# semchan/DCT_Pruning

Measured on NVIDIA B200. Metric: dct_importance_score_images_per_s, higher is better.
Workload: dtype bf16 hi/lo split of fp32 on tcgen05 (fp32 accumulate), fp64 cross-image sums

## Files before the change

### dct_pruning_b200/csrc/dctp.cu

```cuda
#include <cmath>
#include <cstdarg>
#include <cstdio>
#include <cstdlib>
#include <cstring>
#include <map>
#include <mutex>
#include <utility>
#include <vector>

#include "../../include/dctp.h"
#include "score_simt.cuh"
#include "score_large.cuh"
#include "score_tmem.cuh"
#include "score_stack.cuh"
#include "score_kron.cuh"
#include "score_umma.cuh"
#include "topk.cuh"
#include "gather.cuh"
#include "score_alt.cuh"

namespace {

using namespace dctp;

// ... 101 lines not shown
    auto key = std::make_pair(N, KP);
    auto it = g.umma.find(key);
    if (it != g.umma.end()) { out = it->second; return DCTP_OK; }
    const int Ms = (N + 7) / 8 * 8, J = KP / Ms;
    std::vector<uint16_t> hi(static_cast<size_t>(KP) * KP, 0), lo(hi.size(), 0);
    for (int j = 0; j < J; ++j)
        for (int v = 0; v < N; ++v)
            for (int w = 0; w < N; ++w)
                split_bf16(dct_coef(v, w, N), hi[(size_t)(j * Ms + v) * KP + j * Ms + w], lo[(size_t)(j * Ms + v) * KP + j * Ms + w]);
    UmmaBasis b;
    CUDA_TRY(cudaMalloc(&b.hi, hi.size() * 2));
    CUDA_TRY(cudaMalloc(&b.lo, lo.size() * 2));
    CUDA_TRY(cudaMemcpy(b.hi, hi.data(), hi.size() * 2, cudaMemcpyHostToDevice));
    CUDA_TRY(cudaMemcpy(b.lo, lo.data(), lo.size() * 2, cudaMemcpyHostToDevice));
    const int G = 128 / Ms, MT = G * J, NN = N * N;
    if ((MT * NN) % 4 == 0) {
        b.vpe = (N % 4 == 0) ? 1 : (N % 2 == 0) ? 2 : 4;
        b.tile_vec = MT * NN / 4;
        const int step = 4 / b.vpe;
        std::vector<uint16_t> tab(static_cast<size_t>(b.tile_vec) * b.vpe + 8, 0);
        for (int v = 0; v < b.tile_vec; ++v)
            for (int s = 0; s < b.vpe; ++s) {
                const int e = 4 * v + s * step, t = e / NN, r = e % NN;
                tab[(size_t)v * b.vpe + s] =
                    static_cast<uint16_t>(detail::kmajor_off((t / J) * Ms + r / N, (t % J) * Ms + r % N, 128));
            }
        CUDA_TRY(cudaMalloc(&b.scatter, tab.size() * 2));
        CUDA_TRY(cudaMemcpy(b.scatter, tab.data(), tab.size() * 2, cudaMemcpyHostToDevice));
    }
    g.umma[key] = b;
    out = b;
    return DCTP_OK;
}

inline int t_n1max(int N) { return N <= 32 ? 32 : 64; }
inline int t_groups(int N) { return N <= 8 ? 4 : N <= 16 ? 2 : 1; }

int get_t_basis(int N, TBasis& out) {
    auto it = g.tmem.find(N);
    if (it != g.tmem.end()) { out = it->second; return DCTP_OK; }
    const int Ms = (N + 7) / 8 * 8, G = 128 / Ms, NN = N * N, rows = t_n1max(N), J = t_groups(N);
    std::vector<uint32_t> ahi(128 * 64, 0), alo(128 * 64, 0);
    std::vector<uint16_t> chi(64 * 64, 0), clo(64 * 64, 0);
    for (int gI = 0; gI < G; ++gI)
        for (int v = 0; v < N; ++v)
            for (int w = 0; w < N; ++w) {
                uint16_t h, l;
                split_bf16(dct_coef(v, w, N), h, l);
                const int row = gI * Ms + v, k = gI * N + w;
                ahi[row * 64 + k / 2] |= static_cast<uint32_t>(h) << (16 * (k & 1));
                alo[row * 64 + k / 2] |= static_cast<uint32_t>(l) << (16 * (k & 1));
            }
    for (int rep = 0; rep < (Ms == 8 ? 2 : 1); ++rep)
        for (int u = 0; u < N; ++u)
            for (int h = 0; h < N; ++h) split_bf16(dct_coef(u, h, N), chi[(rep * 8 + u) * 64 + rep * 8 + h], clo[(rep * 8 + u) * 64 + rep * 8 + h]);
    TBasis b;
    b.vpe = (N % 4 == 0) ? 1 : (N % 2 == 0) ? 2 : 4;
    b.tile_vec = G * J * NN / 4;
    const int step = 4 / b.vpe;
    std::vector<uint16_t> tab(static_cast<size_t>(b.tile_vec) * b.vpe + 8, 0);
    for (int v = 0; v < b.tile_vec; ++v)
        for (int sI = 0; sI < b.vpe; ++sI) {
            const int e = 4 * v + sI * step, t = e / NN, r = e % NN, gI = t / J, j = t % J;
            tab[(size_t)v * b.vpe + sI] = static_cast<uint16_t>(detail::kmajor_off(j * Ms + r / N, gI * N + r % N, rows));
        }
    CUDA_TRY(cudaMalloc(&b.a_hi, ahi.size() * 4));
    CUDA_TRY(cudaMalloc(&b.a_lo, alo.size() * 4));
    CUDA_TRY(cudaMalloc(&b.c_hi, chi.size() * 2));
    CUDA_TRY(cudaMalloc(&b.c_lo, clo.size() * 2));
    CUDA_TRY(cudaMalloc(&b.scatter, tab.size() * 2));
    CUDA_TRY(cudaMemcpy(b.a_hi, ahi.data(), ahi.size() * 4, cudaMemcpyHostToDevice));
    CUDA_TRY(cudaMemcpy(b.a_lo, alo.data(), alo.size() * 4, cudaMemcpyHostToDevice));
    CUDA_TRY(cudaMemcpy(b.c_hi, chi.data(), chi.size() * 2, cudaMemcpyHostToDevice));
    CUDA_TRY(cudaMemcpy(b.c_lo, clo.data(), clo.size() * 2, cudaMemcpyHostToDevice));
    CUDA_TRY(cudaMemcpy(b.scatter, tab.data(), tab.size() * 2, cudaMemcpyHostToDevice));
    g.tmem[N] = b;
    out = b;
    return DCTP_OK;
}

inline int stack_kp(int N) { return (N + 15) / 16 * 16; }
inline int stack_sets(int kp) { return kp <= 32 ? 64 / kp : 1; }
inline int stack_g(int kp) { return kp == 16 ? 8 : kp == 32 ? 4 : 2; }
bool stack_shape_supported(int N) { return N >= 10 && N <= 64 && (N % 2) == 0 && (N <= 32 || (N % 4) == 0); }

int get_stack_basis(int N, StackBasis& out) {
    auto it = g.stack.find(N);
    if (it != g.stack.end()) { out = it->second; return DCTP_OK; }
    using S = StackSmem;
    const int KP = stack_kp(N), J = stack_sets(KP), G = stack_g(KP), NN = N * N, Np = (N + 7) / 8 * 8, MT = G * J;
    std::vector<uint32_t> img(128 * 32, 0);
    for (int lane = 0; lane < 128; ++lane) {
        const int q = lane >> 5, part = (lane >> 4) & 1, r = lane & 15;
        const int set = J == 4 ? q : J == 2 ? q >> 1 : 0;
        const int v = J == 4 ? r : J == 2 ? 16 * (q & 1) + r : 16 * q + r;
        if (v >= N) continue;
        for (int w = 0; w < N; ++w) {
            uint16_t h, l;
            split_bf16(dct_coef(v, w, N), h, l);
            const int k = set * KP + w;
            img[lane * 32 + k / 2] |= static_cast<uint32_t>(part ? l : h) << (16 * (k & 1));
        }
    }
    std::vector<uint8_t> chi(S::C2_HALF, 0), clo(S::C2_HALF, 0);
    for (int u = 0; u < N; ++u)
        for (int h = 0; h < N; ++h) {
            uint16_t hh, ll;
            split_bf16(dct_coef(u, h, N), hh, ll);
            const size_t off = static_cast<size_t>(h / 8) * S::LBO2 + u * 16 + (h % 8) * 2;
            std::memcpy(&chi[off], &hh, 2);
            std::memcpy(&clo[off], &ll, 2);
        }
    StackBasis b;
    b.kp = KP;
    b.vec = (N % 4) == 0 ? 4 : 2;
    b.tile_vec = MT * NN / 4;
    const int pieces = b.vec == 4 ? 1 : 2;
    std::vector<uint16_t> tab(static_cast<size_t>(b.tile_vec) * pieces + 8, 0);
    auto fill = [&](uint32_t lbo) {
        for (int f = 0; f < b.tile_vec; ++f)
            for (int pc = 0; pc < pieces; ++pc) {
                const int e = 4 * f + 2 * pc, m = e / NN, rem = e % NN, h = rem / N, w = rem % N, gI = m / J, set = m % J;
                const int n = gI * Np + h, k = set * KP + w;
                tab[static_cast<size_t>(f) * pieces + pc] = static_cast<uint16_t>((k / 8) * lbo + n * 16 + (k % 8) * 2);
            }
    };
    auto store_wavefronts = [&]() {
        long long total = 0;
        const int width = b.vec == 4 ? 2 : 1, lanes = b.vec == 4 ? 16 : 32;
        for (int f0 = 0; f0 < b.tile_vec; f0 += lanes)
            for (int pc = 0; pc < pieces; ++pc) {
                int cnt[32] = {0}, worst = 0;
                for (int t = 0; t < lanes && f0 + t < b.tile_vec; ++t)
                    for (int w = 0; w < width; ++w) {
                        const int bank = (tab[static_cast<size_t>(f0 + t) * pieces + pc] / 4 + w) % 32;
                        if (++cnt[bank] > worst) worst = cnt[bank];
                    }
                total += worst;
            }
        return total;
    };
    long long best = -1;
    for (uint32_t u = 0; u < 8; ++u) {
        fill(2048u + 16u * u);
        const long long wf = store_wavefronts();
        if (best < 0 || wf < best) { best = wf; b.lbo1 = 2048u + 16u * u; }
    }
    fill(b.lbo1);
    b.table_bytes = static_cast<uint32_t>((static_cast<size_t>(b.tile_vec) * pieces * 2 + 15) / 16 * 16);
    if (b.table_bytes > S::TABLE_MAX) return fail(DCTP_E_UNSUPPORTED, "stacked-basis kernel: offset table of side %d does not fit", N);
    CUDA_TRY(cudaMalloc(&b.a_img, img.size() * 4));
    CUDA_TRY(cudaMalloc(&b.c2_hi, chi.size()));
    CUDA_TRY(cudaMalloc(&b.c2_lo, clo.size()));
    CUDA_TRY(cudaMalloc(&b.table, tab.size() * 2));
    CUDA_TRY(cudaMemcpy(b.a_img, img.data(), img.size() * 4, cudaMemcpyHostToDevice));
    CUDA_TRY(cudaMemcpy(b.c2_hi, chi.data(), chi.size(), cudaMemcpyHostToDevice));
    CUDA_TRY(cudaMemcpy(b.c2_lo, clo.data(), clo.size(), cudaMemcpyHostToDevice));
    CUDA_TRY(cudaMemcpy(b.table, tab.data(), tab.size() * 2, cudaMemcpyHostToDevice));
    g.stack[N] = b;
    out = b;
    return DCTP_OK;
}

constexpr int STACK_CFGS = 8, STACK_VARIANTS = 10;
typedef void (*StackKernel)(const ScoreTensorMaps, const StackArgs);
template <bool TRACE, int NCONV, int NE1G = 1, int NE2G = 2>
StackKernel stack_kernel_of(int v) {
    switch (v) {
        case 0: return score_stack_kernel<16, 4, NCONV, NE1G, 2, NE2G, 2, TRACE>;
        case 1: return score_stack_kernel<16, 2, NCONV, NE1G, 2, NE2G, 2, TRACE>;
        case 2: return score_stack_kernel<32, 4, NCONV, NE1G, 2, NE2G, 3, TRACE>;
        case 3: return score_stack_kernel<32, 4, NCONV, NE1G, 2, NE2G, 4, TRACE>;
        case 4: return score_stack_kernel<32, 2, NCONV, NE1G, 2, NE2G, 3, TRACE>;
        case 5: return score_stack_kernel<32, 2, NCONV, NE1G, 2, NE2G, 4, TRACE>;
        case 6: return score_stack_kernel<48, 4, NCONV, NE1G, 2, NE2G, 5, TRACE>;
        case 7: return score_stack_kernel<48, 4, NCONV, NE1G, 2, NE2G, 6, TRACE>;
        case 8: return score_stack_kernel<64, 4, NCONV, NE1G, 2, NE2G, 7, TRACE>;
        default: return score_stack_kernel<64, 4, NCONV, NE1G, 2, NE2G, 8, TRACE>;
    }
}
bool stack_cfg_valid(int cfg) { return cfg == 4 || cfg == 6 || cfg == 7; }
StackKernel stack_kernel_fn(int cfg, int v) {
    switch (cfg) {
        case 6: return stack_kernel_of<true, 8>(v);
        case 7: return stack_kernel_of<false, 12>(v);
        default: return stack_kernel_of<false, 8>(v);
    }
}
const void* stack_kernel_ptr(int cfg, int v) { return reinterpret_cast<const void*>(stack_kernel_fn(cfg, v)); }
int stack_threads(int cfg) { return (cfg == 7 ? 31 : 27) * 32; }
int stack_variant(int KP, int vec, int np8) {
    if (KP == 16) return vec == 4 ? 0 : 1;
    if (KP == 32) return (vec == 4 ? 2 : 4) + (np8 == 4 ? 1 : 0);
    if (KP == 48) return np8 == 6 ? 7 : 6;
    return np8 == 8 ? 9 : 8;
}

typedef CUresult (*EncodeTiledFn)(CUtensorMap*, CUtensorMapDataType, cuuint32_t, void*, const cuuint64_t*, const cuuint64_t*, const cuuint32_t*,
                                  const cuuint32_t*, CUtensorMapInterleave, CUtensorMapSwizzle, CUtensorMapL2promotion, CUtensorMapFloatOOBfill);

template <typename Args>
cudaError_t launch_score_tma(void (*kern)(const ScoreTensorMaps, const Args), int grid, int block, size_t smem, cudaStream_t stream,
                             const ScoreTensorMaps& maps, const Args& args);

struct SiteDesc { const float* first; int B; int c_count; double* accum; };

int encode_flat_map(CUtensorMap& map, const float* first, long long total_elems, int box_rows) {
    std::memset(&map, 0, sizeof map);
    const long long rows = total_elems / 32;
    if (rows <= 0) return DCTP_OK;
    cuuint64_t gdim[2] = {32, static_cast<cuuint64_t>(rows)};
    cuuint64_t gstr[1] = {128};
    cuuint32_t box[2] = {32, static_cast<cuuint32_t>(box_rows)}, estr[2] = {1, 1};
    const CUresult r = reinterpret_cast<EncodeTiledFn>(g.encode_tiled)(
        &map, CU_TENSOR_MAP_DATA_TYPE_FLOAT32, 2, const_cast<float*>(first), gdim, gstr, box, estr, CU_TENSOR_MAP_INTERLEAVE_NONE,
        CU_TENSOR_MAP_SWIZZLE_NONE, CU_TENSOR_MAP_L2_PROMOTION_L2_128B, CU_TENSOR_MAP_FLOAT_OOB_FILL_NONE);
    if (r != CUDA_SUCCESS) return fail(DCTP_E_CUDA, "cuTensorMapEncodeTiled failed (%d) for %lld rows, box %d", (int)r, rows, box_rows);
    return DCTP_OK;
}

int fill_segments(ScoreSegments& seg, const SiteDesc* sites, int n, int NN, int maps_per_tile) {
    seg.n_seg = n;
    int tiles = 0;
    for (int i = 0; i < n; ++i) {
        seg.tile0[i] = tiles;
        seg.n_maps[i] = sites[i].B * sites[i].c_count;
        seg.c_count[i] = sites[i].c_count;
        seg.total_elems[i] = static_cast<long long>(seg.n_maps[i]) * NN;
        seg.x[i] = sites[i].first;
        seg.accum[i] = sites[i].accum;
        tiles += (seg.n_maps[i] + maps_per_tile - 1) / maps_per_tile;
    }
    for (int i = n; i <= SCORE_MAX_SEG; ++i) seg.tile0[i] = tiles;
    return tiles;
}

int launch_stack(const SiteDesc* sites, int n, int N, float* energy_out, float* coeff_out, cudaStream_t stream) {
    StackBasis basis;
    int rc = get_stack_basis(N, basis);
    if (rc) return rc;
    StackArgs a;
    std::memset(&a, 0, sizeof a);
    const int KP = basis.kp, J = stack_sets(KP);
    a.N = N; a.NN = N * N; a.Np = (N + 7) / 8 * 8; a.G = stack_g(KP); a.MT = a.G * J;
    a.ncols = a.G * a.Np;
    a.tile_elems = a.MT * a.NN; a.tile_rows = a.tile_elems / 32; a.tile_vec = basis.tile_vec;
    a.num_tiles = fill_segments(a.seg, sites, n, a.NN, a.MT);
    a.idesc1 = umma::make_idesc_bf16(128, a.ncols, false, false);
    a.idesc2 = umma::make_idesc_bf16(128, KP, false, false);
    a.lbo1 = basis.lbo1;
    a.a_img = basis.a_img; a.c2_hi = basis.c2_hi; a.c2_lo = basis.c2_lo; a.table = basis.table; a.table_bytes = basis.table_bytes;
    a.energy_out = n == 1 ? energy_out : nullptr; a.dump = n == 1 ? coeff_out : nullptr; a.status = g.status;
    ScoreTensorMaps maps;
    for (int i = 0; i < n; ++i)
        if ((rc = encode_flat_map(maps.m[i], sites[i].first, a.seg.total_elems[i], a.tile_rows))) return rc;
    for (int i = n; i < SCORE_MAX_SEG; ++i) maps.m[i] = maps.m[0];
    int grid = g.sm_count < a.num_tiles ? g.sm_count : a.num_tiles;
    const size_t smem = StackSmem::TOTAL;
    const bool v4 = basis.vec == 4;
    static long long* trace_buf = nullptr;
    const bool tracing = std::getenv("DCTP_S_TRACE") != nullptr;
    if (tracing) {
        if (!trace_buf) CUDA_TRY(cudaMalloc(&trace_buf, 64 * sizeof(long long)));
        CUDA_TRY(cudaMemset(trace_buf, 0, 64 * sizeof(long long)));
        a.trace = trace_buf;
    }
    const int variant = stack_variant(KP, v4 ? 4 : 2, a.Np / 8);
    const int cfg = (a.energy_out || a.dump || tracing) ? 6 : g.stack_cfg ? g.stack_cfg : 7;
    CUDA_TRY(launch_score_tma(stack_kernel_fn(cfg, variant), grid, stack_threads(cfg), smem, stream, maps, a));
    note_kernel("score_stack_kernel<KP=%d,VEC=%d,cfg%d> (tcgen05, stacked hi/lo basis in TMEM, TMA tile ring, warp specialised)", KP, basis.vec, cfg);
    if (tracing) {
        long long h[64];
        CUDA_TRY(cudaMemcpy(h, trace_buf, sizeof h, cudaMemcpyDeviceToHost));
        const double nt = h[14] > 0 ? double(h[14]) : 1.0;
        fprintf(stderr, "[dctp trace] stack N=%d cfg %d, CTA 0, %lld tiles, cycles per tile | producer: wait slot %.0f | converter: wait Bx free %.0f, "
                        "wait TMA %.0f, convert %.0f, fence+arrive %.0f | issuer 1: wait Bx %.0f, wait D1 free %.0f, issue %.0f | issuer 2: wait A2 %.0f, "
                        "wait D2 free %.0f, issue %.0f | epi1 (first group, per tile of the CTA): wait D1 %.0f, wait A2 free %.0f, work %.0f | "
                        "epi2: wait D2 %.0f, TMEM loads %.0f, sums+shuffles %.0f, atomics %.0f\n",
                N, cfg, h[14], h[0] / nt, h[16] / nt, h[17] / nt, h[18] / nt, h[19] / nt, h[8] / nt, h[9] / nt, h[10] / nt, h[40] / nt,
                h[41] / nt, h[42] / nt, h[24] / nt, h[25] / nt, h[26] / nt, h[32] / nt, h[34] / nt, h[35] / nt, h[33] / nt);
        fprintf(stderr, "[dctp trace] CTA 0, ns since kernel entry: TMEM + barriers ready %lld, bases staged and dependency wait over %lld, tile loop %lld\n", h[52], h[53], h[51]);
        fprintf(stderr, "[dctp trace] tile loop of CTA 0: %lld SM cycles in %lld ns = %.0f MHz, %.0f cycles per tile\n", h[50], h[51],
                h[51] > 0 ? 1e3 * double(h[50]) / double(h[51]) : 0.0, double(h[50]) / nt);
    }
    g.launches += 1;
    CUDA_TRY(cudaGetLastError());
    return DCTP_OK;
}

int get_kron_basis(int N, KronBasis& out) {
    auto it = g.kron.find(N);
    if (it != g.kron.end()) { out = it->second; return DCTP_OK; }
    using S = StackSmem;
    std::vector<uint8_t> hi(S::C2_HALF, 0), lo(S::C2_HALF, 0);
    for (int u = 0; u < N; ++u)
        for (int v = 0; v < N; ++v)
            for (int h = 0; h < N; ++h)
                for (int w = 0; w < N; ++w) {
                    uint16_t hh, ll;
                    split_bf16(dct_coef(u, h, N) * dct_coef(v, w, N), hh, ll);
                    const int n = u * N + v, k = h * N + w;
                    const size_t off = static_cast<size_t>(k / 8) * S::LBO2 + n * 16 + (k % 8) * 2;
                    std::memcpy(&hi[off], &hh, 2);
                    std::memcpy(&lo[off], &ll, 2);
                }
    KronBasis b;
    CUDA_TRY(cudaMalloc(&b.hi, hi.size()));
    CUDA_TRY(cudaMalloc(&b.lo, lo.size()));
    CUDA_TRY(cudaMemcpy(b.hi, hi.data(), hi.size(), cudaMemcpyHostToDevice));
    CUDA_TRY(cudaMemcpy(b.lo, lo.data(), lo.size(), cudaMemcpyHostToDevice));
    g.kron[N] = b;
    out = b;
    return DCTP_OK;
}

int launch_kron(const SiteDesc* sites, int n, int N, float* energy_out, float* coeff_out, cudaStream_t stream) {
    KronBasis basis;
    int rc = get_kron_basis(N, basis);
    if (rc) return rc;
    KronArgs a;
    std::memset(&a, 0, sizeof a);
    const int NN = N * N, K2 = (NN + 15) / 16 * 16;
    const bool even = (N % 2) == 0;
    a.N = N; a.NN = NN;
    a.idesc = umma::make_idesc_bf16(128, K2, false, false);
    a.k_hi = basis.hi; a.k_lo = basis.lo;
    a.energy_out = n == 1 ? energy_out : nullptr; a.dump = n == 1 ? coeff_out : nullptr; a.status = g.status;
    if (even) {
        a.sub_tiles = N == 8 ? 1 : 2;
        a.row_floats = NN + (((NN / 4) % 2) == 0 ? 4 : 0);
        a.tile_maps = 128 * a.sub_tiles;
        a.box_rows = a.tile_maps;
        a.tile_bytes = static_cast<uint32_t>(a.tile_maps) * a.row_floats * 4u;
    } else {
        a.sub_tiles = N == 7 ? 1 : N == 5 ? 2 : 4;
        a.row_floats = NN;
        a.tile_maps = 128 * a.sub_tiles;
        a.box_rows = a.tile_maps * NN / 32;
        a.tile_bytes = static_cast<uint32_t>(a.box_rows) * 128u;
    }
    a.num_tiles = fill_segments(a.seg, sites, n, NN, a.tile_maps);
    ScoreTensorMaps maps;
    for (int i = 0; i < n; ++i) {
        if (even) {
            std::memset(&maps.m[i], 0, sizeof(CUtensorMap));
            cuuint64_t gdim[2] = {static_cast<cuuint64_t>(NN), static_cast<cuuint64_t>(a.seg.n_maps[i])};
            cuuint64_t gstr[1] = {static_cast<cuuint64_t>(NN) * 4};
            cuuint32_t box[2] = {static_cast<cuuint32_t>(a.row_floats), static_cast<cuuint32_t>(a.tile_maps)}, estr[2] = {1, 1};
            const CUresult r = reinterpret_cast<EncodeTiledFn>(g.encode_tiled)(
                &maps.m[i], CU_TENSOR_MAP_DATA_TYPE_FLOAT32, 2, const_cast<float*>(sites[i].first), gdim, gstr, box, estr,
// ... 889 lines not shown
```

### dct_pruning_b200/csrc/score_stack.cuh

```cuda
#pragma once
#include <cuda.h>
#include "score_umma.cuh"

namespace dctp {

constexpr int SCORE_MAX_SEG = 16;

struct ScoreSegments {
    int n_seg;
    int tile0[SCORE_MAX_SEG + 1];
    int n_maps[SCORE_MAX_SEG], c_count[SCORE_MAX_SEG];
    long long total_elems[SCORE_MAX_SEG];
    const float* x[SCORE_MAX_SEG];
    double* accum[SCORE_MAX_SEG];
};
struct ScoreTensorMaps { CUtensorMap m[SCORE_MAX_SEG]; };

struct StackArgs {
    ScoreSegments seg;
    int N, NN, Np;
    int G, MT;
    int ncols;
    int tile_elems, tile_rows, tile_vec, num_tiles;
    uint32_t idesc1, idesc2;
    uint32_t lbo1;
    const uint32_t* a_img;
    const uint8_t* c2_hi;
    const uint8_t* c2_lo;
    const uint16_t* table;
    uint32_t table_bytes;
    float* energy_out;
    float* dump;
    int* status;
    long long* trace;
};

struct StackSmem {
    static constexpr uint32_t NSTG = 3, STG_STRIDE = 32768;
    static constexpr uint32_t LBO1_MAX = 128 * 16 + 16 * 7;
    static constexpr uint32_t BX_HALF = 8 * LBO1_MAX;
    static constexpr uint32_t LBO2 = 64 * 16 + 16;
    static constexpr uint32_t C2_HALF = 8 * LBO2;
    static constexpr uint32_t OFF_BX = NSTG * STG_STRIDE;
    static constexpr uint32_t NBX = 3;
    static constexpr uint32_t OFF_C2 = OFF_BX + 2 * NBX * BX_HALF;
    static constexpr uint32_t OFF_TABLE = OFF_C2 + 2 * C2_HALF;
    static constexpr uint32_t TABLE_MAX = 8192;
    static constexpr uint32_t OFF_RED = OFF_TABLE + TABLE_MAX;
    static constexpr uint32_t OFF_BARS = OFF_RED + 256;
    static constexpr uint32_t OFF_SLOT = OFF_BARS + 256;
    static constexpr uint32_t TOTAL = OFF_SLOT + 128;
};


template <int KP, int VEC, int NCONV, int NE1G, int NCG, int NE2G = 1, int NP8 = 0, bool TRACE = false>
__global__ void __launch_bounds__((NCONV + 8 * NE1G + 4 * NE2G + 3) * 32, 1) score_stack_kernel(const __grid_constant__ ScoreTensorMaps tmaps, const __grid_constant__ StackArgs a) {
    using S = StackSmem;
    using namespace umma;
    constexpr int J = KP <= 32 ? 64 / KP : 1;
    constexpr int K1S = J * KP / 16, K2S = KP / 16;
    constexpr int G = KP == 16 ? 8 : KP == 32 ? 4 : 2, T2 = G / 2;
    constexpr uint32_t W_E1 = NCONV, W_E2 = NCONV + 8 * NE1G, W_PROD = W_E2 + 4 * NE2G, W_MMA = W_PROD + 1, W_MMA2 = W_PROD + 2, NT = (W_MMA2 + 1) * 32;
    constexpr uint32_t NCT = NCONV * 32 / NCG;
    constexpr uint32_t NBXK = KP == 32 ? 2u : 3u;
    constexpr uint32_t TM_A = 0, TM_D1 = 32;
    const uint32_t d1_stride = a.ncols <= 112 ? 112u : 128u;
    const uint32_t TM_A2 = TM_D1 + 2 * d1_stride, TM_D2 = TM_A2 + 128;
    const uint32_t nb2 = TM_D2 + 128 <= 512 ? 2u : 1u;
    const uint32_t STEP1 = (2 * a.lbo1) >> 4;
    constexpr uint32_t STEP2 = (2 * S::LBO2) >> 4;

    extern __shared__ __align__(1024) uint8_t smem[];
    const uint32_t tid = threadIdx.x, warp = __shfl_sync(0xffffffffu, tid >> 5, 0), lane = tid & 31;
    uint8_t* stg = smem;
    uint8_t* bx = smem + S::OFF_BX;
    uint8_t* c2 = smem + S::OFF_C2;
    const uint8_t* tab = smem + S::OFF_TABLE;
    float* red = reinterpret_cast<float*>(smem + S::OFF_RED);
    uint64_t* bars = reinterpret_cast<uint64_t*>(smem + S::OFF_BARS);
    uint64_t* stg_full = bars;
    uint64_t* stg_free = bars + 3;
    uint64_t* bx_full = bars + 6;
    uint64_t* bx_free = bars + 9;
    uint64_t* d1_full = bars + 12;
    uint64_t* d1_free = bars + 14;
    uint64_t* a2_full = bars + 16;
    uint64_t* a2_free = bars + 18;
    uint64_t* d2_full = bars + 20;
    uint64_t* d2_free = bars + 22;
    uint32_t* tmem_slot = reinterpret_cast<uint32_t*>(smem + S::OFF_SLOT);

    long long tr_entry = 0;
    if (TRACE && a.trace != nullptr && blockIdx.x == 0 && threadIdx.x == 0) asm volatile("mov.u64 %0, %%globaltimer;" : "=l"(tr_entry));
    if (warp == W_MMA) tmem_alloc<512>(tmem_slot);
    if (tid == 0) {
        for (int s = 0; s < 3; ++s) { mbar_init(stg_full + s, 1); mbar_init(stg_free + s, NCONV / NCG); }
        for (int b = 0; b < (int)S::NBX; ++b) { mbar_init(bx_full + b, NCONV / NCG); mbar_init(bx_free + b, 1); }
        for (int b = 0; b < 2; ++b) {
            mbar_init(d1_full + b, 1); mbar_init(d1_free + b, 8);
            mbar_init(a2_full + b, 8); mbar_init(a2_free + b, 1);
            mbar_init(d2_full + b, 1); mbar_init(d2_free + b, 4);
        }
        mbar_init_fence();
    }
    if (warp == W_PROD && lane == 0) tma_prefetch_desc(&tmaps.m[0]);
    tc_fence_before_sync();
    __syncthreads();
    tc_fence_after_sync();
    const uint32_t tmem = *tmem_slot;
    launch_dependents();
    if (TRACE && a.trace != nullptr && blockIdx.x == 0 && tid == 0) { long long t_; asm volatile("mov.u64 %0, %%globaltimer;" : "=l"(t_)); a.trace[52] = t_ - tr_entry; }
    if (warp != W_PROD) {
        const uint32_t ptid = tid < W_PROD * 32 ? tid : tid - 32;
        constexpr uint32_t PNT = NT - 32;
        static_assert(2 * PNT * 16 >= S::C2_HALF && PNT * 16 >= S::TABLE_MAX, "prologue loads are unrolled for these sizes");
        uint4 c2h[2], c2l[2], tb = make_uint4(0, 0, 0, 0), ai[8];
#pragma unroll
        for (int i = 0; i < 2; ++i) {
            const uint32_t off = (ptid + i * PNT) * 16;
            if (off < S::C2_HALF) {
                c2h[i] = *reinterpret_cast<const uint4*>(a.c2_hi + off);
                c2l[i] = *reinterpret_cast<const uint4*>(a.c2_lo + off);
            }
        }
        if (ptid * 16 < a.table_bytes) tb = *reinterpret_cast<const uint4*>(reinterpret_cast<const uint8_t*>(a.table) + ptid * 16);
        if (warp < 4) {
#pragma unroll
            for (int i = 0; i < 8; ++i) ai[i] = reinterpret_cast<const uint4*>(a.a_img + tid * 32)[i];
        }
        for (uint32_t off = ptid * 16; off < 2 * S::NBX * S::BX_HALF; off += PNT * 16) *reinterpret_cast<uint4*>(bx + off) = make_uint4(0, 0, 0, 0);
#pragma unroll
        for (int i = 0; i < 2; ++i) {
            const uint32_t off = (ptid + i * PNT) * 16;
            if (off < S::C2_HALF) {
                *reinterpret_cast<uint4*>(c2 + off) = c2h[i];
                *reinterpret_cast<uint4*>(c2 + S::C2_HALF + off) = c2l[i];
            }
        }
        if (ptid * 16 < a.table_bytes) *reinterpret_cast<uint4*>(smem + S::OFF_TABLE + ptid * 16) = tb;
        if (warp < 4) {
#pragma unroll
            for (int part = 0; part < 2; ++part) {
                uint32_t v[16];
#pragma unroll
                for (int i = 0; i < 4; ++i) {
                    const uint4 q4 = ai[4 * part + i];
                    v[4 * i] = q4.x; v[4 * i + 1] = q4.y; v[4 * i + 2] = q4.z; v[4 * i + 3] = q4.w;
                }
                tmem_st16(tmem + ((warp * 32u) << 16) + TM_A + part * 16, v);
            }
            tmem_st_wait();
// ... 130 lines not shown
                if (!tail) ++it;
                continue;
            }
            const uint32_t b = n % NBXK, s = it % S::NSTG;
            TR_START();
            {
                bool ok = true;
                if (n >= NBXK) ok = mbar_wait(bx_free + b, ((n / NBXK) - 1u) & 1u);
                TR_ADD(tr0);
                if (ok && !tail) ok = mbar_wait(stg_full + s, (it / S::NSTG) & 1u);
                TR_ADD(tr1);
                if (!ok) { dead = true; break; }
            }
            uint8_t* hi = bx + b * 2 * S::BX_HALF;
            uint8_t* lo = hi + S::BX_HALF;
            auto emit = [&](uint32_t o, const float4 v) {
                uint32_t h0, l0, h1, l1;
                split2_packed(pack2(__float_as_uint(v.x), __float_as_uint(v.y)), h0, l0);
                split2_packed(pack2(__float_as_uint(v.z), __float_as_uint(v.w)), h1, l1);
                if constexpr (VEC == 4) {
                    *reinterpret_cast<uint2*>(hi + o) = make_uint2(h0, h1);
                    *reinterpret_cast<uint2*>(lo + o) = make_uint2(l0, l1);
                } else {
                    const uint32_t o0 = o & 0xFFFFu, o1 = o >> 16;
                    *reinterpret_cast<uint32_t*>(hi + o0) = h0;
                    *reinterpret_cast<uint32_t*>(lo + o0) = l0;
                    *reinterpret_cast<uint32_t*>(hi + o1) = h1;
                    *reinterpret_cast<uint32_t*>(lo + o1) = l1;
                }
            };
            auto entry = [&](int f) {
                return VEC == 4 ? static_cast<uint32_t>(reinterpret_cast<const uint16_t*>(tab)[f]) : reinterpret_cast<const uint32_t*>(tab)[f];
            };
            if (!tail) {
                const float4* src = reinterpret_cast<const float4*>(stg + s * S::STG_STRIDE);
                constexpr int CB = 3;
                int f0 = ctid;
                for (; f0 + (int)NCT * (CB - 1) < a.tile_vec - (a.tile_vec % (int)NCT) ; f0 += NCT * CB) {
                    float4 v[CB];
                    uint32_t o[CB];
#pragma unroll
                    for (int i = 0; i < CB; ++i) { v[i] = src[f0 + (int)NCT * i]; o[i] = entry(f0 + (int)NCT * i); }
#pragma unroll
                    for (int i = 0; i < CB; ++i) emit(o[i], v[i]);
                }
                {
                    float4 v[CB];
                    uint32_t o[CB];
#pragma unroll
                    for (int i = 0; i < CB; ++i) {
                        const int f = f0 + (int)NCT * i;
                        if (f < a.tile_vec) { v[i] = src[f]; o[i] = entry(f); }
                    }
#pragma unroll
                    for (int i = 0; i < CB; ++i)
                        if (f0 + (int)NCT * i < a.tile_vec) emit(o[i], v[i]);
                }
                TR_ADD(tr2);
                __syncwarp();
                if (lane == 0) mbar_arrive(stg_free + s);
                ++it;
            } else {
                const long long e0 = static_cast<long long>(tile - a.seg.tile0[sg]) * a.tile_elems, total = a.seg.total_elems[sg];
                const float* xs = a.seg.x[sg];
                for (int f = ctid; f < a.tile_vec; f += NCT) {
                    const long long e = e0 + 4ll * f;
                    float4 v;
                    v.x = e + 0 < total ? xs[e + 0] : 0.f;
                    v.y = e + 1 < total ? xs[e + 1] : 0.f;
                    v.z = e + 2 < total ? xs[e + 2] : 0.f;
                    v.w = e + 3 < total ? xs[e + 3] : 0.f;
                    emit(entry(f), v);
                }
            }
            fence_async_smem();
            __syncwarp();
            if (lane == 0) mbar_arrive(bx_full + b);
            TR_ADD(tr3);
        }
        TR_FLUSH(16);
    } else if (warp < W_E2) {
        const uint32_t q = warp & 3u, s = ((warp - W_E1) >> 2) & 1u, eg = (warp - W_E1) >> 3;
        const uint32_t lane_q = (q * 32u) << 16, lane_s = (q * 32u + s * 16u) << 16;
        const int np8 = NP8 ? NP8 : (a.Np >> 3);
        tr_me = tr_on && warp == W_E1 && lane == 0;
        auto convert16 = [&](const uint32_t (&za)[8], const uint32_t (&zb)[8], uint32_t dst_hi, uint32_t dst_lo) {
            uint32_t h[4], l[4];
#pragma unroll
            for (int i = 0; i < 4; ++i)
                split2_packed(add2_packed(pack2(za[2 * i], za[2 * i + 1]), pack2(zb[2 * i], zb[2 * i + 1])), h[i], l[i]);
            tmem_st_frag8(dst_hi, h);
            tmem_st_frag8(dst_lo, l);
        };
        uint32_t n = eg;
        for (int tile = first + (int)eg * stride; tile < a.num_tiles; tile += NE1G * stride, n += NE1G) {
            const uint32_t b = n & 1u;
            const uint32_t d1 = tmem + TM_D1 + b * d1_stride;
            TR_START();
            {
                bool ok = true;
                ok = mbar_wait(d1_full + b, (n >> 1) & 1u);
                TR_ADD(tr0);
                if (ok && n >= 2) ok = mbar_wait(a2_free + b, ((n >> 1) - 1u) & 1u);
                TR_ADD(tr1);
                if (!ok) { dead = true; break; }
            }
            tc_fence_after_sync();
            constexpr int CPT = KP / 16, NCH = T2 * CPT;
#pragma unroll
            for (int ch0 = 0; ch0 < NCH; ch0 += 2) {
                uint32_t za[16], zb[16];
#pragma unroll
                for (int k = 0; k < 2; ++k) {
                    const int ch = ch0 + k;
                    if (ch < NCH) {
                        const int t = ch / CPT, c8 = 2 * (ch % CPT);
                        const uint32_t src_a = d1 + lane_q + (2 * t + s) * a.Np + c8 * 8, src_b = src_a + (16u << 16);
                        if (c8 + 2 <= np8) {
                            tmem_ld_frag16(src_a, reinterpret_cast<uint32_t (&)[8]>(za[8 * k]));
                            tmem_ld_frag16(src_b, reinterpret_cast<uint32_t (&)[8]>(zb[8 * k]));
                        } else if (c8 < np8) {
                            tmem_ld_frag8(src_a, reinterpret_cast<uint32_t (&)[4]>(za[8 * k]));
                            tmem_ld_frag8(src_b, reinterpret_cast<uint32_t (&)[4]>(zb[8 * k]));
                        }
                    }
                }
                tmem_ld_wait();
                if (ch0 + 2 >= NCH) {
                    tc_fence_before_sync();
                    __syncwarp();
                    if (lane == 0) mbar_arrive(d1_free + b);
                }
#pragma unroll
                for (int k = 0; k < 2; ++k) {
                    const int ch = ch0 + k;
                    if (ch < NCH) {
                        const int t = ch / CPT, c8 = 2 * (ch % CPT);
                        const uint32_t dst_hi = tmem + TM_A2 + b * 64 + t * KP + lane_s + c8 * 4, dst_lo = dst_hi + KP / 2;
                        if (c8 + 2 <= np8) {
                            convert16(reinterpret_cast<const uint32_t (&)[8]>(za[8 * k]), reinterpret_cast<const uint32_t (&)[8]>(zb[8 * k]), dst_hi, dst_lo);
                        } else if (c8 < np8) {
                            uint32_t h[2], l[2];
#pragma unroll
                            for (int i = 0; i < 2; ++i)
                                split2_packed(add2_packed(pack2(za[8 * k + 2 * i], za[8 * k + 2 * i + 1]), pack2(zb[8 * k + 2 * i], zb[8 * k + 2 * i + 1])),
                                              h[i], l[i]);
                            tmem_st_frag4(dst_hi, h[0], h[1]);
                            tmem_st_frag4(dst_lo, l[0], l[1]);
                        }
                    }
                }
            }
            tmem_st_wait();
            tc_fence_before_sync();
            __syncwarp();
            if (lane == 0) mbar_arrive(a2_full + b);
            TR_ADD(tr2);
        }
        TR_FLUSH(24);
    } else if (warp < W_PROD) {
        const uint32_t q = warp & 3u, eg2 = (warp - W_E2) >> 2, et = tid - (W_E2 + 4 * eg2) * 32;
        const uint32_t lane_q = (q * 32u) << 16;
        const uint32_t s = lane >> 4, r = lane & 15u;
        const uint32_t my_set = J == 4 ? q : J == 2 ? (q >> 1) : 0u;
        const uint32_t my_v = J == 4 ? r : J == 2 ? 16u * (q & 1u) + r : 16u * q + r;
        uint32_t n = eg2;
        int sg = 0, chan_sg = -1;
        uint32_t chan0 = 0, chan_step = 0;
        tr_me = tr_on && warp == W_E2 && lane == 0;
        for (int tile = first + (int)eg2 * stride; tile < a.num_tiles; tile += NE2G * stride, n += NE2G) {
            seg_of(tile, sg);
            const uint32_t C = static_cast<uint32_t>(a.seg.c_count[sg]), seg_maps = static_cast<uint32_t>(a.seg.n_maps[sg]);
            double* const accum = a.seg.accum[sg];
            const uint32_t pb = n & 1u, b2 = nb2 == 2 ? pb : 0u;
            TR_START();
            if (!mbar_wait(d2_full + pb, (n >> 1) & 1u)) { dead = true; break; }
            TR_ADD(tr0);
            tc_fence_after_sync();
            const uint32_t d2 = tmem + TM_D2 + b2 * 64 + lane_q;
            const uint32_t m0 = static_cast<uint32_t>(tile - a.seg.tile0[sg]) * a.MT;
            if (sg != chan_sg) {
                chan_sg = sg;
                chan0 = m0 % C;
                chan_step = (static_cast<uint32_t>(NE2G * stride) * static_cast<uint32_t>(a.MT)) % C;
            } else {
                chan0 += chan_step;
                if (chan0 >= C) chan0 -= C;
            }
            float e[T2];
            constexpr int TOT = T2 * KP, HALF = TOT >= 32 ? 32 : TOT;
            float part[4] = {0.f, 0.f, 0.f, 0.f};
#pragma unroll
            for (int c0 = 0; c0 < TOT; c0 += HALF) {
                uint32_t z[HALF];
#pragma unroll
                for (int c = 0; c < HALF; c += 16)
                    if (c0 + c < TOT) tmem_ld16(d2 + c0 + c, reinterpret_cast<uint32_t (&)[16]>(z[c]));
                tmem_ld_wait();
                if (c0 + HALF >= TOT) {
                    tc_fence_before_sync();
                    __syncwarp();
                    if (lane == 0) mbar_arrive(d2_free + pb);
                    TR_ADD(tr2);
                }
#pragma unroll
                for (int c = 0; c < HALF; c += 16) {
                    if (c0 + c < TOT) {
                        const int t = (c0 + c) / KP;
                        float p0 = 0.f, p1 = 0.f, p2 = 0.f, p3 = 0.f;
#pragma unroll
                        for (int i = 0; i < 4; ++i) {
                            p0 = fmaf(__uint_as_float(z[c + i]), __uint_as_float(z[c + i]), p0);
                            p1 = fmaf(__uint_as_float(z[c + 4 + i]), __uint_as_float(z[c + 4 + i]), p1);
                            p2 = fmaf(__uint_as_float(z[c + 8 + i]), __uint_as_float(z[c + 8 + i]), p2);
                            p3 = fmaf(__uint_as_float(z[c + 12 + i]), __uint_as_float(z[c + 12 + i]), p3);
                        }
                        const float p = (p0 + p1) + (p2 + p3);
                        if (T2 == 4) part[t] += p;
                        else if (T2 == 2) part[t] += p;
                        else part[0] += p;
                        if (TRACE && a.dump != nullptr) {
                            const uint32_t m = m0 + (2 * t + s) * J + my_set;
                            const int u0 = (c0 + c) - t * KP;
                            if (m < seg_maps && my_v < (uint32_t)a.N)
#pragma unroll
                                for (int i = 0; i < 16; ++i)
                                    if (u0 + i < a.N) a.dump[static_cast<long long>(m) * a.NN + (u0 + i) * a.N + my_v] = __uint_as_float(z[c + i]);
                        }
                    }
                }
            }
// ... 71 lines not shown
```

Baseline: 122,200.

## Tighten TMEM map pitch per side length and specialise stacked kernel per pitch

New measurement: 126,200 (median of 6 runs). 1.03x the previous value.

```diff
diff --git a/dct_pruning_b200/csrc/dctp.cu b/dct_pruning_b200/csrc/dctp.cu
--- a/dct_pruning_b200/csrc/dctp.cu
+++ b/dct_pruning_b200/csrc/dctp.cu
@@ -207,13 +207,14 @@
 inline int stack_kp(int N) { return (N + 15) / 16 * 16; }
 inline int stack_sets(int kp) { return kp <= 32 ? 64 / kp : 1; }
 inline int stack_g(int kp) { return kp == 16 ? 8 : kp == 32 ? 4 : 2; }
+inline int stack_pitch(int N) { const int r = stack_kp(N) == 16 ? 16 : 16 / stack_g(stack_kp(N)); return (N + r - 1) / r * r; }
 bool stack_shape_supported(int N) { return N >= 10 && N <= 64 && (N % 2) == 0 && (N <= 32 || (N % 4) == 0); }
 
 int get_stack_basis(int N, StackBasis& out) {
     auto it = g.stack.find(N);
     if (it != g.stack.end()) { out = it->second; return DCTP_OK; }
     using S = StackSmem;
-    const int KP = stack_kp(N), J = stack_sets(KP), G = stack_g(KP), NN = N * N, Np = (N + 7) / 8 * 8, MT = G * J;
+    const int KP = stack_kp(N), J = stack_sets(KP), G = stack_g(KP), NN = N * N, Np = stack_pitch(N), MT = G * J;
     std::vector<uint32_t> img(128 * 32, 0);
     for (int lane = 0; lane < 128; ++lane) {
         const int q = lane >> 5, part = (lane >> 4) & 1, r = lane & 15;
@@ -287,21 +288,25 @@
     return DCTP_OK;
 }
 
-constexpr int STACK_CFGS = 8, STACK_VARIANTS = 10;
+constexpr int STACK_CFGS = 8, STACK_VARIANTS = 14;
 typedef void (*StackKernel)(const ScoreTensorMaps, const StackArgs);
 template <bool TRACE, int NCONV, int NE1G = 1, int NE2G = 2>
 StackKernel stack_kernel_of(int v) {
     switch (v) {
-        case 0: return score_stack_kernel<16, 4, NCONV, NE1G, 2, NE2G, 2, TRACE>;
-        case 1: return score_stack_kernel<16, 2, NCONV, NE1G, 2, NE2G, 2, TRACE>;
-        case 2: return score_stack_kernel<32, 4, NCONV, NE1G, 2, NE2G, 3, TRACE>;
-        case 3: return score_stack_kernel<32, 4, NCONV, NE1G, 2, NE2G, 4, TRACE>;
-        case 4: return score_stack_kernel<32, 2, NCONV, NE1G, 2, NE2G, 3, TRACE>;
-        case 5: return score_stack_kernel<32, 2, NCONV, NE1G, 2, NE2G, 4, TRACE>;
-        case 6: return score_stack_kernel<48, 4, NCONV, NE1G, 2, NE2G, 5, TRACE>;
-        case 7: return score_stack_kernel<48, 4, NCONV, NE1G, 2, NE2G, 6, TRACE>;
-        case 8: return score_stack_kernel<64, 4, NCONV, NE1G, 2, NE2G, 7, TRACE>;
-        default: return score_stack_kernel<64, 4, NCONV, NE1G, 2, NE2G, 8, TRACE>;
+        case 0: return score_stack_kernel<16, 2, NCONV, NE1G, 2, NE2G, 16, TRACE>;
+        case 1: return score_stack_kernel<16, 4, NCONV, NE1G, 2, NE2G, 16, TRACE>;
+        case 2: return score_stack_kernel<32, 2, NCONV, NE1G, 2, NE2G, 20, TRACE>;
+        case 3: return score_stack_kernel<32, 4, NCONV, NE1G, 2, NE2G, 20, TRACE>;
+        case 4: return score_stack_kernel<32, 2, NCONV, NE1G, 2, NE2G, 24, TRACE>;
+        case 5: return score_stack_kernel<32, 4, NCONV, NE1G, 2, NE2G, 24, TRACE>;
+        case 6: return score_stack_kernel<32, 2, NCONV, NE1G, 2, NE2G, 28, TRACE>;
+        case 7: return score_stack_kernel<32, 4, NCONV, NE1G, 2, NE2G, 28, TRACE>;
+        case 8: return score_stack_kernel<32, 2, NCONV, NE1G, 2, NE2G, 32, TRACE>;
+        case 9: return score_stack_kernel<32, 4, NCONV, NE1G, 2, NE2G, 32, TRACE>;
+        case 10: return score_stack_kernel<48, 4, NCONV, NE1G, 2, NE2G, 40, TRACE>;
+        case 11: return score_stack_kernel<48, 4, NCONV, NE1G, 2, NE2G, 48, TRACE>;
+        case 12: return score_stack_kernel<64, 4, NCONV, NE1G, 2, NE2G, 56, TRACE>;
+        default: return score_stack_kernel<64, 4, NCONV, NE1G, 2, NE2G, 64, TRACE>;
     }
 }
 bool stack_cfg_valid(int cfg) { return cfg == 4 || cfg == 6 || cfg == 7; }
@@ -314,11 +319,9 @@
 }
 const void* stack_kernel_ptr(int cfg, int v) { return reinterpret_cast<const void*>(stack_kernel_fn(cfg, v)); }
 int stack_threads(int cfg) { return (cfg == 7 ? 31 : 27) * 32; }
-int stack_variant(int KP, int vec, int np8) {
-    if (KP == 16) return vec == 4 ? 0 : 1;
-    if (KP == 32) return (vec == 4 ? 2 : 4) + (np8 == 4 ? 1 : 0);
-    if (KP == 48) return np8 == 6 ? 7 : 6;
-    return np8 == 8 ? 9 : 8;
+int stack_variant(int N) {
+    if (N <= 16) return N % 4 == 0 ? 1 : 0;
+    return N <= 32 ? 2 + (N - 18) / 2 : 10 + (N - 33) / 8;
 }
 
 typedef CUresult (*EncodeTiledFn)(CUtensorMap*, CUtensorMapDataType, cuuint32_t, void*, const cuuint64_t*, const cuuint64_t*, const cuuint32_t*,
@@ -367,7 +370,7 @@
     StackArgs a;
     std::memset(&a, 0, sizeof a);
     const int KP = basis.kp, J = stack_sets(KP);
-    a.N = N; a.NN = N * N; a.Np = (N + 7) / 8 * 8; a.G = stack_g(KP); a.MT = a.G * J;
+    a.N = N; a.NN = N * N; a.Np = stack_pitch(N); a.G = stack_g(KP); a.MT = a.G * J;
     a.ncols = a.G * a.Np;
     a.tile_elems = a.MT * a.NN; a.tile_rows = a.tile_elems / 32; a.tile_vec = basis.tile_vec;
     a.num_tiles = fill_segments(a.seg, sites, n, a.NN, a.MT);
@@ -382,7 +385,6 @@
     for (int i = n; i < SCORE_MAX_SEG; ++i) maps.m[i] = maps.m[0];
     int grid = g.sm_count < a.num_tiles ? g.sm_count : a.num_tiles;
     const size_t smem = StackSmem::TOTAL;
-    const bool v4 = basis.vec == 4;
     static long long* trace_buf = nullptr;
     const bool tracing = std::getenv("DCTP_S_TRACE") != nullptr;
     if (tracing) {
@@ -390,7 +392,7 @@
         CUDA_TRY(cudaMemset(trace_buf, 0, 64 * sizeof(long long)));
         a.trace = trace_buf;
     }
-    const int variant = stack_variant(KP, v4 ? 4 : 2, a.Np / 8);
+    const int variant = stack_variant(N);
     const int cfg = (a.energy_out || a.dump || tracing) ? 6 : g.stack_cfg ? g.stack_cfg : 7;
     CUDA_TRY(launch_score_tma(stack_kernel_fn(cfg, variant), grid, stack_threads(cfg), smem, stream, maps, a));
     note_kernel("score_stack_kernel<KP=%d,VEC=%d,cfg%d> (tcgen05, stacked hi/lo basis in TMEM, TMA tile ring, warp specialised)", KP, basis.vec, cfg);
diff --git a/dct_pruning_b200/csrc/score_stack.cuh b/dct_pruning_b200/csrc/score_stack.cuh
--- a/dct_pruning_b200/csrc/score_stack.cuh
+++ b/dct_pruning_b200/csrc/score_stack.cuh
@@ -53,7 +53,7 @@
 };
 
 
-template <int KP, int VEC, int NCONV, int NE1G, int NCG, int NE2G = 1, int NP8 = 0, bool TRACE = false>
+template <int KP, int VEC, int NCONV, int NE1G, int NCG, int NE2G, int NP, bool TRACE = false>
 __global__ void __launch_bounds__((NCONV + 8 * NE1G + 4 * NE2G + 3) * 32, 1) score_stack_kernel(const __grid_constant__ ScoreTensorMaps tmaps, const __grid_constant__ StackArgs a) {
     using S = StackSmem;
     using namespace umma;
@@ -64,9 +64,10 @@
     constexpr uint32_t NCT = NCONV * 32 / NCG;
     constexpr uint32_t NBXK = KP == 32 ? 2u : 3u;
     constexpr uint32_t TM_A = 0, TM_D1 = 32;
-    const uint32_t d1_stride = a.ncols <= 112 ? 112u : 128u;
-    const uint32_t TM_A2 = TM_D1 + 2 * d1_stride, TM_D2 = TM_A2 + 128;
-    const uint32_t nb2 = TM_D2 + 128 <= 512 ? 2u : 1u;
+    static_assert(NP % 4 == 0 && G * NP % 16 == 0 && NP <= KP, "map pitch: see stack_pitch");
+    constexpr uint32_t d1_stride = G * NP <= 112 ? 112u : 128u;
+    constexpr uint32_t TM_A2 = TM_D1 + 2 * d1_stride, TM_D2 = TM_A2 + 128;
+    constexpr uint32_t nb2 = TM_D2 + 128 <= 512 ? 2u : 1u;
     const uint32_t STEP1 = (2 * a.lbo1) >> 4;
     constexpr uint32_t STEP2 = (2 * S::LBO2) >> 4;
 
@@ -363,16 +364,7 @@
     } else if (warp < W_E2) {
         const uint32_t q = warp & 3u, s = ((warp - W_E1) >> 2) & 1u, eg = (warp - W_E1) >> 3;
         const uint32_t lane_q = (q * 32u) << 16, lane_s = (q * 32u + s * 16u) << 16;
-        const int np8 = NP8 ? NP8 : (a.Np >> 3);
         tr_me = tr_on && warp == W_E1 && lane == 0;
-        auto convert16 = [&](const uint32_t (&za)[8], const uint32_t (&zb)[8], uint32_t dst_hi, uint32_t dst_lo) {
-            uint32_t h[4], l[4];
-#pragma unroll
-            for (int i = 0; i < 4; ++i)
-                split2_packed(add2_packed(pack2(za[2 * i], za[2 * i + 1]), pack2(zb[2 * i], zb[2 * i + 1])), h[i], l[i]);
-            tmem_st_frag8(dst_hi, h);
-            tmem_st_frag8(dst_lo, l);
-        };
         uint32_t n = eg;
         for (int tile = first + (int)eg * stride; tile < a.num_tiles; tile += NE1G * stride, n += NE1G) {
             const uint32_t b = n & 1u;
@@ -387,7 +379,9 @@
                 if (!ok) { dead = true; break; }
             }
             tc_fence_after_sync();
-            constexpr int CPT = KP / 16, NCH = T2 * CPT;
+            constexpr int CPT = KP / 16, NCH = T2 * CPT, NPC = (NP + 7) / 8;
+            auto piece = [](int i) { return 8 * i + 8 <= NP ? 8 * i : NP - 8; };
+            auto fused = [&](int i) { return i + 1 < NPC && piece(i + 1) == piece(i) + 8; };
 #pragma unroll
             for (int ch0 = 0; ch0 < NCH; ch0 += 2) {
                 uint32_t za[16], zb[16];
@@ -395,14 +389,18 @@
                 for (int k = 0; k < 2; ++k) {
                     const int ch = ch0 + k;
                     if (ch < NCH) {
-                        const int t = ch / CPT, c8 = 2 * (ch % CPT);
-                        const uint32_t src_a = d1 + lane_q + (2 * t + s) * a.Np + c8 * 8, src_b = src_a + (16u << 16);
-                        if (c8 + 2 <= np8) {
-                            tmem_ld_frag16(src_a, reinterpret_cast<uint32_t (&)[8]>(za[8 * k]));
-                            tmem_ld_frag16(src_b, reinterpret_cast<uint32_t (&)[8]>(zb[8 * k]));
-                        } else if (c8 < np8) {
-                            tmem_ld_frag8(src_a, reinterpret_cast<uint32_t (&)[4]>(za[8 * k]));
-                            tmem_ld_frag8(src_b, reinterpret_cast<uint32_t (&)[4]>(zb[8 * k]));
+                        const int t = ch / CPT, i = 2 * (ch % CPT);
+                        const uint32_t src_a = d1 + lane_q + (2 * t + s) * NP, src_b = src_a + (16u << 16);
+                        if (fused(i)) {
+                            tmem_ld_frag16(src_a + piece(i), reinterpret_cast<uint32_t (&)[8]>(za[8 * k]));
+                            tmem_ld_frag16(src_b + piece(i), reinterpret_cast<uint32_t (&)[8]>(zb[8 * k]));
+                        } else if (i < NPC) {
+                            tmem_ld_frag8(src_a + piece(i), reinterpret_cast<uint32_t (&)[4]>(za[8 * k]));
+                            tmem_ld_frag8(src_b + piece(i), reinterpret_cast<uint32_t (&)[4]>(zb[8 * k]));
+                            if (i + 1 < NPC) {
+                                tmem_ld_frag8(src_a + piece(i + 1), reinterpret_cast<uint32_t (&)[4]>(za[8 * k + 4]));
+                                tmem_ld_frag8(src_b + piece(i + 1), reinterpret_cast<uint32_t (&)[4]>(zb[8 * k + 4]));
+                            }
                         }
                     }
                 }
@@ -415,19 +413,26 @@
 #pragma unroll
                 for (int k = 0; k < 2; ++k) {
                     const int ch = ch0 + k;
-                    if (ch < NCH) {
-                        const int t = ch / CPT, c8 = 2 * (ch % CPT);
-                        const uint32_t dst_hi = tmem + TM_A2 + b * 64 + t * KP + lane_s + c8 * 4, dst_lo = dst_hi + KP / 2;
-                        if (c8 + 2 <= np8) {
-                            convert16(reinterpret_cast<const uint32_t (&)[8]>(za[8 * k]), reinterpret_cast<const uint32_t (&)[8]>(zb[8 * k]), dst_hi, dst_lo);
-                        } else if (c8 < np8) {
-                            uint32_t h[2], l[2];
-#pragma unroll
-                            for (int i = 0; i < 2; ++i)
-                                split2_packed(add2_packed(pack2(za[8 * k + 2 * i], za[8 * k + 2 * i + 1]), pack2(zb[8 * k + 2 * i], zb[8 * k + 2 * i + 1])),
-                                              h[i], l[i]);
-                            tmem_st_frag4(dst_hi, h[0], h[1]);
-                            tmem_st_frag4(dst_lo, l[0], l[1]);
+                    const int t = ch / CPT, i = 2 * (ch % CPT);
+                    if (ch < NCH && i < NPC) {
+                        const uint32_t dst_hi = tmem + TM_A2 + b * 64 + t * KP + lane_s, dst_lo = dst_hi + KP / 2;
+                        const int npairs = i + 1 < NPC ? 4 : 2;
+                        uint32_t h[4], l[4];
+#pragma unroll
+                        for (int j = 0; j < 4; ++j)
+                            if (j < npairs)
+                                split2_packed(add2_packed(pack2(za[8 * k + 2 * j], za[8 * k + 2 * j + 1]), pack2(zb[8 * k + 2 * j], zb[8 * k + 2 * j + 1])),
+                                              h[j], l[j]);
+                        if (fused(i)) {
+                            tmem_st_frag8(dst_hi + piece(i) / 2, h);
+                            tmem_st_frag8(dst_lo + piece(i) / 2, l);
+                        } else {
+                            tmem_st_frag4(dst_hi + piece(i) / 2, h[0], h[1]);
+                            tmem_st_frag4(dst_lo + piece(i) / 2, l[0], l[1]);
+                            if (i + 1 < NPC) {
+                                tmem_st_frag4(dst_hi + piece(i + 1) / 2, h[2], h[3]);
+                                tmem_st_frag4(dst_lo + piece(i + 1) / 2, l[2], l[3]);
+                            }
                         }
                     }
                 }
```
